# muzishen/IMAGHarmony

Hardware: AMD Instinct MI355X
Metric: 1024^2 SDXL images/sec (30 DDIM steps, PNS N seeds) (higher is better)
Workload: dtype bf16

## Files before the change

### imagharmony_amd/csrc/attention.hip

```cpp
#include "imh_attn_core.h"

namespace imh {

int g_attn_force_nw = 0;
int g_attn_mode = 0;
constexpr float ATT_DEFER_LOG2 = 8.0f;

template <typename T, int NW, int NPASS>
__global__ __launch_bounds__(64 * NW, (NPASS == 1 && NW == 4) ? 3 : 2) void attn_kernel(const AttnParams p) {
    constexpr int RND = 8 / NW;
    typedef typename Vec<T>::v8 v8;
    typedef typename Vec<T>::v4 v4;
    static_assert(32 * NW * 128 <= ATT_STAGES * 2 * ATT_TILE_BYTES, "Q/O staging must fit inside the ring");
    __shared__ __attribute__((aligned(16))) unsigned char smem[ATT_STAGES * 2 * ATT_TILE_BYTES];
    unsigned char* qs = smem;

    const int tid = threadIdx.x;
    const int lane = tid & 63;
    const int wave = __builtin_amdgcn_readfirstlane(tid >> 6);
    const int l32 = lane & 31;
    const int hi = lane >> 5;
    const int gx = (p.Lq + 32 * NW - 1) / (32 * NW);
    const int items = gx * p.H * p.B;
    const int per = (items + 7) >> 3;
    const int item = (blockIdx.x & 7) * per + (blockIdx.x >> 3);
    if ((int)(blockIdx.x >> 3) >= per || item >= items) return;
    const int hb = item / gx, qblk = item - hb * gx;
    const int b = hb / p.H, h = hb - b * p.H;
    const int q0 = qblk * (32 * NW);
    const int q = q0 + wave * 32 + l32;

    v8 qf[4];
    {
#pragma unroll
        for (int i = 0; i < 4; ++i) {
            const int row = wave * 32 + i * 8 + (lane >> 3);
            const int ch = stage_chunk_x(row, lane);
            const T* src = (const T*)p.Q + ((size_t)b * p.Lq + min(q0 + row, p.Lq - 1)) * p.ldq + h * 64 + ch * 8;
            glds16(src, qs + (wave * 32 + i * 8) * 128);
        }
        asm volatile("s_waitcnt vmcnt(0)" ::: "memory");
        const int row = wave * 32 + l32;
#pragma unroll
        for (int sd = 0; sd < 4; ++sd) qf[sd] = *(const v8*)(qs + tile_off(row, sd * 2 + hi, swz_x(row)));
        asm volatile("s_waitcnt lgkmcnt(0)" ::: "memory");
        __builtin_amdgcn_s_barrier();
    }

    f32x16 fin[2];
    attn_core<T, NW, NPASS>(p, smem, qf, b, h, wave, lane, item, fin);
    attn_store<T, NW>(p, qs, fin, b, h, q0, wave, lane);
    if (!ATT_TIMING) tail_prefetch(p.pf_ptr, p.pf_bytes, item, items, tid, 64 * NW);
}


template <typename T>
__global__ __launch_bounds__(256, 2) void attn_pipe_kernel(const AttnParams p) {
    constexpr int NW = 4;
    typedef typename Vec<T>::v8 v8;
    extern __shared__ __attribute__((aligned(16))) unsigned char smem[];
    unsigned char* qs = smem;
    const int tid = threadIdx.x;
    const int lane = tid & 63;
    const int wave = __builtin_amdgcn_readfirstlane(tid >> 6);
    const int l32 = lane & 31;
    const int hi = lane >> 5;
    const int gx = (p.Lq + 32 * NW - 1) / (32 * NW);
    const int items = gx * p.H * p.B;
    const int per = (items + 7) >> 3;
    const int split = p.split;
    const int jx = blockIdx.x >> 3;
    int item, qg = -1;
    if (jx < per - split) item = (blockIdx.x & 7) * per + jx;
    else {
        const int k = jx - (per - split);
        if (k >= 4 * split) return;
        item = (blockIdx.x & 7) * per + (per - split) + (k >> 2);
        qg = k & 3;
    }
    if (item >= items) return;
    const int hb = item / gx, qblk = item - hb * gx;
    const int b = hb / p.H, h = hb - b * p.H;
    const int q0 = qblk * (32 * NW);
#if ATT_TIMING == 2
    const unsigned long long ts_entry_ = __builtin_amdgcn_s_memrealtime();
#endif
    if (qg >= 0) {
        const float c = p.scale * LOG2E;
        unsigned char* my = smem + wave * (2 * ATT_TILE_BYTES);
        v8 qf[4];
        {
            const T* qrow = (const T*)p.Q + ((size_t)b * p.Lq + q0 + qg * 32 + l32) * p.ldq + h * 64 + hi * 8;
#pragma unroll
            for (int sd = 0; sd < 4; ++sd) qf[sd] = *(const v8*)(qrow + sd * 16);
        }
        f32x16 o[2];
#pragma unroll
        for (int dt = 0; dt < 2; ++dt)
#pragma unroll
            for (int r = 0; r < 16; ++r) o[dt][r] = 0.f;
        float m_run = NEG_BIG, l_run = 0.f;
        const int ntq = (p.Lk / ATT_KV) >> 2;
        const unsigned char* kq[2];
        const unsigned char* vq[2];
#pragma unroll
        for (int par = 0; par < 2; ++par) {
            const int row = par * 8 + (lane >> 3);
            const int ch = stage_chunk_x(row, lane);
            kq[par] = (const unsigned char*)((const T*)p.K + ((size_t)b * p.Lk_pad + row) * p.ldk + h * 64 + ch * 8);
            vq[par] = (const unsigned char*)((const T*)p.Vt + ((size_t)h * 64 + row) * p.ldvt + (size_t)b * p.Lk_pad + ch * 8);
        }
        const size_t kstep = (size_t)ATT_KV * p.ldk * sizeof(T), vstep = (size_t)ATT_KV * sizeof(T);
        const size_t krow16 = (size_t)16 * p.ldk * sizeof(T), vrow16 = (size_t)16 * p.ldvt * sizeof(T);
        for (int t = 0; t < ntq; ++t) {
            const int tile = wave * ntq + t;
#pragma unroll
            for (int i = 0; i < 2; ++i)
#pragma unroll
                for (int w = 0; w < 4; ++w) {
                    const int g16 = i * 2 + (w >> 1);
                    glds16(kq[w & 1] + tile * kstep + g16 * krow16, my + (i * 32 + w * 8) * 128);
                    glds16(vq[w & 1] + tile * vstep + g16 * vrow16, my + ATT_TILE_BYTES + (i * 32 + w * 8) * 128);
                }
            asm volatile("s_waitcnt vmcnt(0)" ::: "memory");
            attn_tile<T, false>(my, my + ATT_TILE_BYTES, qf, lane, tile * ATT_KV, p.Lk, c, o, m_run, l_run);
            asm volatile("s_waitcnt lgkmcnt(0)" ::: "memory");
        }
        const float l_tot = l_run + __shfl_xor(l_run, 32, 64);
        if (wave > 0) {
            float* w = (float*)my;
#pragma unroll
            for (int dt = 0; dt < 2; ++dt)
#pragma unroll
                for (int r = 0; r < 16; ++r) w[(dt * 16 + r) * 64 + lane] = o[dt][r];
            w[32 * 64 + lane] = m_run;
            w[33 * 64 + lane] = l_tot;
        }
        asm volatile("s_waitcnt lgkmcnt(0)" ::: "memory");
        __builtin_amdgcn_s_barrier();
        asm volatile("" ::: "memory");
        if (wave == 0) {
            float mi[4], li[4];
            mi[0] = m_run; li[0] = l_tot;
#pragma unroll
            for (int g = 1; g < 4; ++g) {
                const float* w = (const float*)(smem + g * (2 * ATT_TILE_BYTES));
                mi[g] = w[32 * 64 + lane]; li[g] = w[33 * 64 + lane];
            }
            const float m = fmaxf(fmaxf(mi[0], mi[1]), fmaxf(mi[2], mi[3]));
            float ai[4], den = 0.f;
#pragma unroll
            for (int g = 0; g < 4; ++g) { ai[g] = __builtin_amdgcn_exp2f((mi[g] - m) * c); den += li[g] * ai[g]; }
            const float inv = 1.0f / den;
            f32x16 fin[2];
#pragma unroll
            for (int dt = 0; dt < 2; ++dt)
#pragma unroll
                for (int r = 0; r < 16; ++r) {
                    float v = o[dt][r] * ai[0];
#pragma unroll
                    for (int g = 1; g < 4; ++g) v += ((const float*)(smem + g * (2 * ATT_TILE_BYTES)))[(dt * 16 + r) * 64 + lane] * ai[g];
                    fin[dt][r] = v * inv;
                }
            attn_store<T, 1>(p, smem, fin, b, h, q0 + qg * 32, 0, lane);
        }
#if ATT_TIMING == 2
        if (tid == 0 && p.pf_ptr) {
            asm volatile("s_waitcnt vmcnt(0)" ::: "memory");
            unsigned hwid;
            asm volatile("s_getreg_b32 %0, hwreg(HW_REG_HW_ID)" : "=s"(hwid));
            unsigned long long* dbg = (unsigned long long*)p.pf_ptr + (size_t)blockIdx.x * 4;
            dbg[0] = ts_entry_; dbg[1] = __builtin_amdgcn_s_memrealtime(); dbg[2] = hwid; dbg[3] = (blockIdx.x & 7) | 0x100;
        }
#else
        if (qg == 0) tail_prefetch(p.pf_ptr, p.pf_bytes, item, items, tid, 64 * NW);
#endif
        return;
    }
    v8 qf[4];
    {
#pragma unroll
        for (int i = 0; i < 4; ++i) {
            const int row = wave * 32 + i * 8 + (lane >> 3);
            const int ch = stage_chunk_x(row, lane);
            const T* src = (const T*)p.Q + ((size_t)b * p.Lq + min(q0 + row, p.Lq - 1)) * p.ldq + h * 64 + ch * 8;
            glds16(src, qs + (wave * 32 + i * 8) * 128);
        }
        asm volatile("s_waitcnt vmcnt(0)" ::: "memory");
        const int row = wave * 32 + l32;
#pragma unroll
        for (int sd = 0; sd < 4; ++sd) qf[sd] = *(const v8*)(qs + tile_off(row, sd * 2 + hi, swz_x(row)));
        asm volatile("s_waitcnt lgkmcnt(0)" ::: "memory");
        __builtin_amdgcn_s_barrier();
    }
    f32x16 fin[2];
    attn_core_pipe<T>(p, smem, qf, b, h, wave, lane, fin);
    attn_store<T, NW>(p, qs, fin, b, h, q0, wave, lane);
#if ATT_TIMING == 2
    if (tid == 0 && p.pf_ptr) {
        asm volatile("s_waitcnt vmcnt(0)" ::: "memory");
        unsigned hwid;
        asm volatile("s_getreg_b32 %0, hwreg(HW_REG_HW_ID)" : "=s"(hwid));
        unsigned long long* dbg = (unsigned long long*)p.pf_ptr + (size_t)blockIdx.x * 4;
        dbg[0] = ts_entry_; dbg[1] = __builtin_amdgcn_s_memrealtime(); dbg[2] = hwid; dbg[3] = blockIdx.x & 7;
    }
#else
    tail_prefetch(p.pf_ptr, p.pf_bytes, item, items, tid, 64 * NW);
#endif
}

#ifdef IMH_EXPERIMENTAL
template <typename T>
__global__ __launch_bounds__(512, 4) void attn_ks_kernel(const AttnParams p) {
    typedef typename Vec<T>::v8 v8;
    extern __shared__ __attribute__((aligned(16))) unsigned char smem[];
    const int tid = threadIdx.x;
    const int lane = tid & 63;
    const int wave = __builtin_amdgcn_readfirstlane(tid >> 6);
    const int g = wave >> 2, qg = wave & 3;
    const int hi = lane >> 5;
    const int gx = (p.Lq + 127) / 128;
    const int items = gx * p.H * p.B;
    const int per = (items + 7) >> 3;
    const int item = (blockIdx.x & 7) * per + (blockIdx.x >> 3);
    if ((int)(blockIdx.x >> 3) >= per || item >= items) return;
    const int hb = item / gx, qblk = item - hb * gx;
    const int b = hb / p.H, h = hb - b * p.H;
    const int q0 = qblk * 128;
    v8 qf[4];
    {
        const T* qrow = (const T*)p.Q + ((size_t)b * p.Lq + min(q0 + qg * 32 + (lane & 31), p.Lq - 1)) * p.ldq + h * 64 + hi * 8;
#pragma unroll
        for (int sd = 0; sd < 4; ++sd) qf[sd] = *(const v8*)(qrow + sd * 16);
    }
    f32x16 o[2], fin[2];
    float m_run, l_run;
    attn_core_ks<T>(p, smem + g * (2 * 2 * ATT_TILE_BYTES), qf, b, h, g, qg, lane, o, m_run, l_run);
    asm volatile("s_waitcnt lgkmcnt(0)" ::: "memory");
    __builtin_amdgcn_s_barrier();
    attn_ks_merge((float*)smem, p.scale * LOG2E, g, qg, lane, o, m_run, l_run, fin);
    if (g == 0) attn_store<T, 4>(p, smem + 4 * 34 * 64 * 4, fin, b, h, q0, qg, lane);
    else tail_prefetch(p.pf_ptr, p.pf_bytes, item, items, tid - 256, 256);
}
#endif

template <typename T>
__global__ __launch_bounds__(256) void attn_small_kernel(const SmallAttnParams p) {
    extern __shared__ float sm[];
    float* sc = sm;
    float* qrow = sm + p.Lk;
    float* red = qrow + p.dq;
    const int b = blockIdx.x / p.H, h = blockIdx.x % p.H;
    const int tid = threadIdx.x;
    const T* Q = (const T*)p.Q + (size_t)b * p.Lq * p.ldq + h * p.dq;
    const T* K = (const T*)p.K + (size_t)b * p.Lk * p.ldk + h * p.dq;
    const T* V = (const T*)p.V + (size_t)b * p.Lk * p.ldv + h * p.dv;
    T* O = (T*)p.O + (size_t)b * p.Lq * p.ldo + h * p.dv;
    for (int i = 0; i < p.Lq; ++i) {
        for (int d = tid; d < p.dq; d += 256) qrow[d] = to_f32(Q[(size_t)i * p.ldq + d]);
        __syncthreads();
        float mx = -1e30f;
        for (int k = tid; k < p.Lk; k += 256) {
            const T* kr = K + (size_t)k * p.ldk;
            float s = 0.f;
            for (int d = 0; d < p.dq; ++d) s += qrow[d] * to_f32(kr[d]);
            s *= p.scale;
            sc[k] = s;
            mx = fmaxf(mx, s);
        }
        mx = wave_max(mx);
        if ((tid & 63) == 0) red[tid >> 6] = mx;
        __syncthreads();
        mx = fmaxf(fmaxf(red[0], red[1]), fmaxf(red[2], red[3]));
        float sum = 0.f;
        for (int k = tid; k < p.Lk; k += 256) { const float e = __expf(sc[k] - mx); sc[k] = e; sum += e; }
        sum = wave_sum(sum);
        if ((tid & 63) == 0) red[4 + (tid >> 6)] = sum;
        __syncthreads();
        sum = red[4] + red[5] + red[6] + red[7];
// ... 55 lines not shown
        for (int k0 = 0; k0 < LkP; k0 += 64) {
            const int k = k0 + lane;
            const float e = k < p.Lk ? __expf(mypr[k] - mx) : 0.f;
            mypr[k] = e;
            sum += e;
        }
        sum = wave_sum(sum);
        __builtin_amdgcn_wave_barrier();
        const float inv = 1.0f / sum;
        for (int d = lane; d < p.dv; d += 64) {
            float o = 0.f;
            for (int k = 0; k < p.Lk; ++k) o += mypr[k] * to_f32(vs[(size_t)k * p.dv + d]);
            O[(size_t)q * p.ldo + d] = from_f32<T>(o * inv);
        }
        __builtin_amdgcn_wave_barrier();
    }
}

int attention_small_launch(const SmallAttnParams& p, int dtype, hipStream_t stream) {
    if (p.B <= 0 || p.H <= 0 || p.Lq <= 0 || p.Lk <= 0 || p.dq <= 0 || p.dv <= 0 || p.Lk > 8192 || p.dq > 1024) {
        set_error("attention_small: unsupported shape"); return IMH_ERR_SHAPE;
    }
    if (dtype != IMH_DT_BF16 && dtype != IMH_DT_F16) { set_error("attention_small: unknown dtype %d", dtype); return IMH_ERR_DTYPE; }
    {
        const int LkP = (p.Lk + 63) & ~63;
        const size_t need = ((size_t)p.dq * LkP + (size_t)p.Lk * p.dv) * 2 + (size_t)(4 * LkP + 4 * p.dq) * sizeof(float);
        const bool aligned = !(p.dq & 7) && !(p.dv & 7) && !(p.ldk & 7) && !(p.ldv & 7) && !(((size_t)p.Lk * p.dv * 2 + (size_t)p.dq * LkP * 2) & 15);
        if (aligned && need <= 150 * 1024) {
            dim3 grid(p.B * p.H);
            if (dtype == IMH_DT_BF16) {
                static DynLdsOnce a0;
                a0.ensure((const void*)attn_small_lds_kernel<bf16_t>, 150 * 1024);
                hipLaunchKernelGGL((attn_small_lds_kernel<bf16_t>), grid, dim3(256), need, stream, p, LkP);
            } else {
                static DynLdsOnce a1;
                a1.ensure((const void*)attn_small_lds_kernel<f16_t>, 150 * 1024);
                hipLaunchKernelGGL((attn_small_lds_kernel<f16_t>), grid, dim3(256), need, stream, p, LkP);
            }
            return check_launch("attn_small_lds_kernel");
        }
    }
    const size_t lds = (size_t)(p.Lk + p.dq + 8) * sizeof(float);
    dim3 grid(p.B * p.H);
    if (dtype == IMH_DT_BF16) hipLaunchKernelGGL((attn_small_kernel<bf16_t>), grid, dim3(256), lds, stream, p);
    else if (dtype == IMH_DT_F16) hipLaunchKernelGGL((attn_small_kernel<f16_t>), grid, dim3(256), lds, stream, p);
    else { set_error("attention_small: unknown dtype %d", dtype); return IMH_ERR_DTYPE; }
    return check_launch("attn_small_kernel");
}

int attention_launch(const AttnParams& p, int dtype, hipStream_t stream) {
    if (p.Lk <= 0 || p.Lk_pad % ATT_KV != 0 || p.Lk_pad < p.Lk) {
        set_error("attention: Lk=%d Lk_pad=%d (pad must be a multiple of 64 and >= Lk)", p.Lk, p.Lk_pad);
        return IMH_ERR_SHAPE;
    }
    if (p.K2 && (p.Lk2 <= 0 || p.Lk2_pad % ATT_KV != 0 || p.Lk2_pad < p.Lk2)) {
        set_error("attention: Lk2=%d Lk2_pad=%d invalid", p.Lk2, p.Lk2_pad);
        return IMH_ERR_SHAPE;
    }
    if ((p.ldq & 7) || (p.ldk & 7) || (p.ldvt & 7) || (p.ldo & 7) || (p.K2 && ((p.ldk2 & 7) || (p.ldvt2 & 7)))) {
        set_error("attention: leading dimensions must be multiples of 8 elements");
        return IMH_ERR_SHAPE;
    }
    if (p.B <= 0 || p.H <= 0 || p.Lq <= 0) { set_error("attention: empty problem"); return IMH_ERR_SHAPE; }
    if (dtype != IMH_DT_BF16 && dtype != IMH_DT_F16) { set_error("attention: unknown dtype %d", dtype); return IMH_ERR_DTYPE; }
    constexpr int nw = 4;
    const int items = ((p.Lq + 32 * nw - 1) / (32 * nw)) * p.H * p.B;
    dim3 grid(8 * ((items + 7) / 8));
    if (!p.K2 && p.Lk % (2 * ATT_KV) == 0 && p.Lk >= 4 * ATT_KV && (g_attn_mode == 5 || g_attn_mode == 6)) {
#ifndef IMH_EXPERIMENTAL
        return experimental_refused("the key-split attention kernel (imh_debug_set(4, 5 | 6))");
#else
        const int lds = 2 * 2 * 2 * ATT_TILE_BYTES;
        const int items128 = ((p.Lq + 127) / 128) * p.H * p.B;
        dim3 grid2(8 * ((items128 + 7) / 8));
        AttnParams q = p;
        q.defer_log2 = g_attn_mode == 6 ? 0.0f : ATT_DEFER_LOG2;
        if (dtype == IMH_DT_BF16) { static DynLdsOnce once; once.ensure((const void*)attn_ks_kernel<bf16_t>, lds);
                                    hipLaunchKernelGGL((attn_ks_kernel<bf16_t>), grid2, dim3(512), lds, stream, q); }
        else { static DynLdsOnce once; once.ensure((const void*)attn_ks_kernel<f16_t>, lds);
               hipLaunchKernelGGL((attn_ks_kernel<f16_t>), grid2, dim3(512), lds, stream, q); }
        return check_launch("attn_ks_kernel");
#endif
    }
    if (!p.K2 && p.Lk % ATT_KV == 0 && (g_attn_mode == 2 || g_attn_mode == 3 || g_attn_mode == 7 || (g_attn_mode == 0 && p.Lk >= 4 * ATT_KV))) {
        const int lds = ATT_PIPE_STAGES * 2 * ATT_TILE_BYTES;
        AttnParams q = p;
        q.defer_log2 = g_attn_mode == 2 ? 0.0f : ATT_DEFER_LOG2;
        const int per = (items + 7) / 8;
        q.split = (g_attn_mode != 7 && per > 32 && per % 32 != 0 && per % 32 <= 16 && p.Lq % 128 == 0 && p.Lk % (4 * ATT_KV) == 0) ? per % 32 : 0;
        dim3 gridp(8 * (per + 3 * q.split));
        if (dtype == IMH_DT_BF16) { static DynLdsOnce once; once.ensure((const void*)attn_pipe_kernel<bf16_t>, lds);
                                    hipLaunchKernelGGL((attn_pipe_kernel<bf16_t>), gridp, dim3(256), lds, stream, q); }
        else { static DynLdsOnce once; once.ensure((const void*)attn_pipe_kernel<f16_t>, lds);
               hipLaunchKernelGGL((attn_pipe_kernel<f16_t>), gridp, dim3(256), lds, stream, q); }
        return check_launch("attn_pipe_kernel");
    }
#define IMH_ATT_LAUNCH(TT, NWV) do { if (p.K2) hipLaunchKernelGGL((attn_kernel<TT, NWV, 2>), grid, dim3(64 * NWV), 0, stream, p); \
        else hipLaunchKernelGGL((attn_kernel<TT, NWV, 1>), grid, dim3(64 * NWV), 0, stream, p); } while (0)
    if (dtype == IMH_DT_BF16) IMH_ATT_LAUNCH(bf16_t, 4);
    else IMH_ATT_LAUNCH(f16_t, 4);
#undef IMH_ATT_LAUNCH
    return check_launch("attn_kernel");
}

}
```

### imagharmony_amd/csrc/imh_attn_core.h

```cpp
#pragma once
#include "imh_common.h"
#include "imh_kernels.h"
#include <type_traits>

namespace imh {

constexpr int ATT_KV = 64;
constexpr int ATT_TILE_BYTES = 64 * 128;
constexpr int ATT_STAGES = 3;
constexpr float LOG2E = 1.4426950408889634f;
constexpr float NEG_BIG = -1.0e30f;

typedef __attribute__((ext_vector_type(2))) float f32x2;
__device__ __forceinline__ float max3f(float a, float b, float c) {
    float r;
    asm("v_max3_f32 %0, %1, %2, %3" : "=v"(r) : "v"(a), "v"(b), "v"(c));
    return r;
}
__device__ __forceinline__ float mfma_first_max(float a, float b) { return __builtin_fmaxf(a, b); }
__device__ __forceinline__ float xhalf_max(float x) {
    const unsigned u = __builtin_bit_cast(unsigned, x);
    auto r = __builtin_amdgcn_permlane32_swap(u, u, false, false);
    return fmaxf(__builtin_bit_cast(float, (unsigned)r[0]), __builtin_bit_cast(float, (unsigned)r[1]));
}
#ifndef ATT_ABL
#define ATT_ABL 0
#endif
#define ATT_EXP2(x) ((ATT_ABL & 9) ? (x) : __builtin_amdgcn_exp2f(x))
#ifndef ATT_TIMING
#define ATT_TIMING 0
#endif
#if ATT_TIMING
#define ATT_TICK(i) do { asm volatile("s_nop 0" ::: "memory"); const unsigned long long tn_ = __builtin_readcyclecounter(); tacc[i] += tn_ - tm0; tm0 = tn_; } while (0)
#else
#define ATT_TICK(i) do {} while (0)
#endif


template <typename T, bool MASK, int NKT>
__device__ __forceinline__ void attn_tile_n(const unsigned char* ks, const unsigned char* vs, const typename Vec<T>::v8 (&qf)[4],
                                            const int lane, const int kbase, const int Lk, const float c, f32x16 (&o)[2],
                                            float& m_run, float& l_run);

template <typename T, int NW, int NPASS>
__device__ __forceinline__ void attn_core(const AttnParams& p, unsigned char* smem, const typename Vec<T>::v8 (&qf)[4],
                                          const int b, const int h, const int wave, const int lane, const int item,
                                          f32x16 (&fin)[2]) {
    constexpr int RND = 8 / NW;
    typedef typename Vec<T>::v8 v8;
    const int tid = threadIdx.x;
    const int hi = lane >> 5;
    (void)tid; (void)item;
    const float c = p.scale * LOG2E;

#pragma unroll
    for (int dt = 0; dt < 2; ++dt)
#pragma unroll
        for (int r = 0; r < 16; ++r) fin[dt][r] = 0.f;

#pragma unroll
    for (int pass = 0; pass < NPASS; ++pass) {
        const T* Kp = (const T*)(pass == 0 ? p.K : p.K2);
        const T* Vp = (const T*)(pass == 0 ? p.Vt : p.Vt2);
        const int Lk = pass == 0 ? p.Lk : p.Lk2;
        const int Lkp = pass == 0 ? p.Lk_pad : p.Lk2_pad;
        const int ldk = pass == 0 ? p.ldk : p.ldk2;
        const int ldvt = pass == 0 ? p.ldvt : p.ldvt2;
        const float wgt = pass == 0 ? 1.0f : (p.scale2_tab ? p.scale2_tab[*p.step] : p.scale2);
        const int ntiles = (Lk + ATT_KV - 1) / ATT_KV;

        auto stage = [&](int buf, int tile) {
            unsigned char* ks = smem + buf * 2 * ATT_TILE_BYTES;
            unsigned char* vs = ks + ATT_TILE_BYTES;
            const int kbase = tile * ATT_KV;
#pragma unroll
            for (int i = 0; i < RND; ++i) {
                const int row = i * (NW * 8) + wave * 8 + (lane >> 3);
                const int ch = stage_chunk_x(row, lane);
                const T* ksrc = Kp + ((size_t)b * Lkp + kbase + row) * ldk + h * 64 + ch * 8;
                glds16(ksrc, ks + (i * (NW * 8) + wave * 8) * 128);
                const T* vsrc = Vp + ((size_t)h * 64 + row) * ldvt + (size_t)b * Lkp + kbase + ch * 8;
                glds16(vsrc, vs + (i * (NW * 8) + wave * 8) * 128);
            }
        };

        f32x16 o[2];
#pragma unroll
        for (int dt = 0; dt < 2; ++dt)
#pragma unroll
            for (int r = 0; r < 16; ++r) o[dt][r] = 0.f;
        float m_run = NEG_BIG, l_run = 0.f;

        constexpr int LPT = 2 * RND;
#pragma unroll
        for (int s = 0; s < ATT_STAGES - 1; ++s)
            if (s < ntiles) stage(s, s);
        int cur = 0;
#if ATT_TIMING
        unsigned long long tacc[5] = {0, 0, 0, 0, 0}, tm0 = __builtin_readcyclecounter();
#endif
        for (int t = 0; t < ntiles; ++t) {
            if (ATT_ABL & 16) {
            } else if (t + ATT_STAGES - 2 < ntiles) asm volatile("s_waitcnt vmcnt(%0)" ::"n"((ATT_STAGES - 2) * LPT) : "memory");
            else asm volatile("s_waitcnt vmcnt(0)" ::: "memory");
            if (!(ATT_ABL & 4)) __builtin_amdgcn_s_barrier();
            asm volatile("" ::: "memory");
// ... 145 lines not shown
        for (int s = 0; s < 2; ++s)
#pragma unroll
            for (int dt = 0; dt < 2; ++dt) vf[kt][s][dt] = *(const v8*)(vs + att_v_off(lane, dt, kt, s));
    __builtin_amdgcn_sched_barrier(0);
    if (ragged) {
#pragma unroll
        for (int kt = 0; kt < NKT; ++kt)
#pragma unroll
            for (int r = 0; r < 16; ++r)
                if (kbase + kt * 32 + st_key(r, hi) >= Lk) st[kt][r] = NEG_BIG;
    }
    float mx;
    if constexpr (NKT == 2) {
        mx = max3f(mfma_first_max(st[0][0], st[1][0]), st[0][1], st[1][1]);
        mx = fmaxf(mx, st[0][2]);
#pragma unroll
        for (int r = 2; r < 15; ++r) mx = max3f(mx, st[1][r], st[0][r + 1]);
        mx = fmaxf(mx, st[1][15]);
    } else {
        mx = max3f(mfma_first_max(st[0][0], st[0][1]), st[0][2], st[0][3]);
#pragma unroll
        for (int r = 4; r < 16; r += 2) mx = max3f(mx, st[0][r], st[0][r + 1]);
    }
    mx = xhalf_max(mx);
    const float m_new = fmaxf(m_run, mx);
    const f32x2 c2 = {c, c};
    const f32x2 nmc2 = {-m_new * c, -m_new * c};
    f32x2 ps2 = {0.f, 0.f};
    v8 pf[NKT][2];
#pragma unroll
    for (int kt = 0; kt < NKT; ++kt)
#pragma unroll
        for (int r = 0; r < 16; r += 2) {
            const f32x2 s2 = {st[kt][r], st[kt][r + 1]};
            const f32x2 e2 = __builtin_elementwise_fma(s2, c2, nmc2);
            const f32x2 p2 = {__builtin_amdgcn_exp2f(e2[0]), __builtin_amdgcn_exp2f(e2[1])};
            ps2 += p2;
            pf[kt][r >> 3][r & 7] = from_f32<T>(p2[0]);
            pf[kt][r >> 3][(r & 7) + 1] = from_f32<T>(p2[1]);
        }
    if (__any(m_new != m_run)) {
        const float alpha = __builtin_amdgcn_exp2f((m_run - m_new) * c);
        l_run *= alpha;
#pragma unroll
        for (int dt = 0; dt < 2; ++dt)
#pragma unroll
            for (int r = 0; r < 16; ++r) o[dt][r] *= alpha;
        m_run = m_new;
    }
    l_run += ps2[0] + ps2[1];
    __builtin_amdgcn_sched_barrier(0);
#pragma unroll
    for (int kt = 0; kt < NKT; ++kt)
#pragma unroll
        for (int s = 0; s < 2; ++s)
#pragma unroll
            for (int dt = 0; dt < 2; ++dt) o[dt] = mfma32(vf[kt][s][dt], pf[kt][s], o[dt]);
}

template <typename T, bool MASK = true>
__device__ __forceinline__ void attn_tile(const unsigned char* ks, const unsigned char* vs, const typename Vec<T>::v8 (&qf)[4],
                                          const int lane, const int kbase, const int Lk, const float c, f32x16 (&o)[2],
                                          float& m_run, float& l_run) {
    if (MASK && kbase + 32 >= Lk) attn_tile_n<T, MASK, 1>(ks, vs, qf, lane, kbase, Lk, c, o, m_run, l_run);
    else attn_tile_n<T, MASK, 2>(ks, vs, qf, lane, kbase, Lk, c, o, m_run, l_run);
}

template <typename T>
__device__ __forceinline__ void attn_stage_tile(const T* Kp, const T* Vp, const int Lkp, const int ldk, const int ldvt, const int b,
                                                const int h, const int tile, unsigned char* ks, unsigned char* vs, const int wave,
                                                const int lane) {
    const int kbase = tile * ATT_KV;
#pragma unroll
    for (int i = 0; i < 2; ++i) {
        const int row = i * 32 + wave * 8 + (lane >> 3);
        const int ch = stage_chunk_x(row, lane);
        glds16(Kp + ((size_t)b * Lkp + kbase + row) * ldk + h * 64 + ch * 8, ks + (i * 32 + wave * 8) * 128);
        glds16(Vp + ((size_t)h * 64 + row) * ldvt + (size_t)b * Lkp + kbase + ch * 8, vs + (i * 32 + wave * 8) * 128);
    }
}

constexpr int ATT_PIPE_STAGES = 4;

template <typename T>
__device__ __forceinline__ void attn_core_pipe(const AttnParams& p, unsigned char* smem, const typename Vec<T>::v8 (&qf)[4],
                                               const int b, const int h, const int wave, const int lane, f32x16 (&fin)[2]) {
    typedef typename Vec<T>::v8 v8;
    constexpr int S = ATT_PIPE_STAGES, LPT = 4;
    const int hi = lane >> 5;
    const float c = p.scale * LOG2E;
    const T* Kp = (const T*)p.K;
    const T* Vp = (const T*)p.Vt;
    const int Lk = p.Lk;
    const int ntiles = (Lk + ATT_KV - 1) / ATT_KV;
    auto stage = [&](int tile) {
        unsigned char* ks = smem + (tile & (S - 1)) * 2 * ATT_TILE_BYTES;
        attn_stage_tile<T>(Kp, Vp, p.Lk_pad, p.ldk, p.ldvt, b, h, tile, ks, ks + ATT_TILE_BYTES, wave, lane);
    };
    const int srow = wave * 8 + (lane >> 3);
    const unsigned char* ksrc[2];
    const unsigned char* vsrc[2];
#pragma unroll
    for (int i = 0; i < 2; ++i) {
        const int row = i * 32 + srow;
        const int ch = stage_chunk_x(row, lane);
        ksrc[i] = (const unsigned char*)(Kp + ((size_t)b * p.Lk_pad + row) * p.ldk + h * 64 + ch * 8);
        vsrc[i] = (const unsigned char*)(Vp + ((size_t)h * 64 + row) * p.ldvt + (size_t)b * p.Lk_pad + ch * 8);
    }
    const size_t kstep = (size_t)ATT_KV * p.ldk * sizeof(T), vstep = (size_t)ATT_KV * sizeof(T);
    auto stage_piece = [&](int tile, int q) {
        unsigned char* ks = smem + (tile & (S - 1)) * 2 * ATT_TILE_BYTES;
        const int i = q >> 1;
        if (q & 1) glds16(vsrc[i] + (size_t)tile * vstep, ks + ATT_TILE_BYTES + (i * 32 + wave * 8) * 128);
        else glds16(ksrc[i] + (size_t)tile * kstep, ks + (i * 32 + wave * 8) * 128);
    };
    f32x16 o[2];
#pragma unroll
    for (int dt = 0; dt < 2; ++dt)
#pragma unroll
        for (int r = 0; r < 16; ++r) o[dt][r] = 0.f;
    float m_run = NEG_BIG, l_run = 0.f;

    auto qk = [&](f32x16 (&st)[2], const unsigned char* ks) {
        v8 kf[2][4];
#pragma unroll
        for (int kt = 0; kt < 2; ++kt)
#pragma unroll
            for (int sd = 0; sd < 4; ++sd) kf[kt][sd] = *(const v8*)(ks + att_k_off(lane, kt, sd));
#pragma unroll
        for (int kt = 0; kt < 2; ++kt) {
#pragma unroll
            for (int r = 0; r < 16; ++r) st[kt][r] = 0.f;
#pragma unroll
            for (int sd = 0; sd < 4; ++sd) st[kt] = mfma32(kf[kt][sd], qf[sd], st[kt]);
        }
    };
    auto rowmax = [&](f32x16 (&st)[2], const int tile) -> float {
        (void)tile; (void)hi;
        float mx = max3f(mfma_first_max(st[0][0], st[1][0]), st[0][1], st[1][1]);
        mx = fmaxf(mx, st[0][2]);
#pragma unroll
        for (int r = 2; r < 15; ++r) mx = max3f(mx, st[1][r], st[0][r + 1]);
        mx = fmaxf(mx, st[1][15]);
        return xhalf_max(mx);
    };
    const float defer = p.defer_log2;
    auto rescale = [&](const float m_new) {
        if (__any((m_new - m_run) * c > defer)) {
            const float alpha = __builtin_amdgcn_exp2f((m_run - m_new) * c);
            l_run *= alpha;
#pragma unroll
            for (int dt = 0; dt < 2; ++dt)
#pragma unroll
                for (int r = 0; r < 16; ++r) o[dt][r] *= alpha;
            m_run = m_new;
        }
    };

#pragma unroll
    for (int s = 0; s < S - 1; ++s)
        if (s < ntiles) stage(s);
    if (ntiles >= 3) asm volatile("s_waitcnt vmcnt(%0)" ::"n"(2 * LPT) : "memory");
    else if (ntiles == 2) asm volatile("s_waitcnt vmcnt(%0)" ::"n"(LPT) : "memory");
    else asm volatile("s_waitcnt vmcnt(0)" ::: "memory");
    __builtin_amdgcn_s_barrier();
    asm volatile("" ::: "memory");
    f32x16 stA[2], stB[2];
    qk(stA, smem);
    rescale(fmaxf(m_run, rowmax(stA, 0)));

    auto iter = [&](auto HN, auto STG, f32x16 (&cur)[2], f32x16 (&nxt)[2], const int t) {
        constexpr bool has_next = decltype(HN)::value;
        constexpr int stg = decltype(STG)::value;
        const bool stage_more = stg == 1 || (stg == 2 && has_next && t + 3 < ntiles);
        if (has_next) {
            if (t + 2 < ntiles) asm volatile("s_waitcnt vmcnt(%0)" ::"n"(LPT) : "memory");
            else asm volatile("s_waitcnt vmcnt(0)" ::: "memory");
            __builtin_amdgcn_s_barrier();
            asm volatile("" ::: "memory");
        }
        const unsigned char* vs = smem + (t & (S - 1)) * 2 * ATT_TILE_BYTES + ATT_TILE_BYTES;
        const unsigned char* ksn = smem + ((t + 1) & (S - 1)) * 2 * ATT_TILE_BYTES;
        v8 kf[2][4], vf[2][2][2];
        if (has_next) {
#pragma unroll
            for (int sd = 0; sd < 4; ++sd)
#pragma unroll
                for (int kt = 0; kt < 2; ++kt) kf[kt][sd] = *(const v8*)(ksn + att_k_off(lane, kt, sd));
        }
        auto v_reads = [&]() {
#pragma unroll
            for (int kt = 0; kt < 2; ++kt)
#pragma unroll
                for (int s2 = 0; s2 < 2; ++s2)
#pragma unroll
                    for (int dt = 0; dt < 2; ++dt) vf[kt][s2][dt] = *(const v8*)(vs + att_v_off(lane, dt, kt, s2));
        };
        if (!has_next) v_reads();
        __builtin_amdgcn_sched_barrier(0);
        const f32x2 c2 = {c, c};
        const f32x2 nmc2 = {-m_run * c, -m_run * c};
        f32x2 ps2 = {0.f, 0.f};
        v8 pf[2][2];
        auto p_chunk = [&](auto J) {
            constexpr int j = decltype(J)::value;
            constexpr int kt = j >> 2, r0 = (j & 3) * 4;
#pragma unroll
            for (int r = r0; r < r0 + 4; r += 2) {
                const f32x2 s2 = {cur[kt][r], cur[kt][r + 1]};
                const f32x2 e2 = __builtin_elementwise_fma(s2, c2, nmc2);
                const f32x2 p2 = {__builtin_amdgcn_exp2f(e2[0]), __builtin_amdgcn_exp2f(e2[1])};
                ps2 += p2;
                pf[kt][r >> 3][r & 7] = from_f32<T>(p2[0]);
                pf[kt][r >> 3][(r & 7) + 1] = from_f32<T>(p2[1]);
            }
        };
        auto b_step = [&](auto J) {
            constexpr int j = decltype(J)::value;
            constexpr int sd = j >> 1, kt = j & 1;
            p_chunk(J);
            if constexpr (j == 3) { if (has_next) v_reads(); }
            __builtin_amdgcn_sched_barrier(0);
            if (has_next) {
                if constexpr (sd == 0) {
#pragma unroll
                    for (int r = 0; r < 16; ++r) nxt[kt][r] = 0.f;
                }
                nxt[kt] = mfma32(kf[kt][sd], qf[sd], nxt[kt]);
                __builtin_amdgcn_sched_barrier(0);
            }
        };
        b_step(std::integral_constant<int, 0>{}); b_step(std::integral_constant<int, 1>{});
        b_step(std::integral_constant<int, 2>{}); b_step(std::integral_constant<int, 3>{});
        b_step(std::integral_constant<int, 4>{}); b_step(std::integral_constant<int, 5>{});
        b_step(std::integral_constant<int, 6>{}); b_step(std::integral_constant<int, 7>{});
        l_run += ps2[0] + ps2[1];
        float mx = NEG_BIG;
        __builtin_amdgcn_sched_barrier(0);
        auto a_step = [&](auto J) {
            constexpr int j = decltype(J)::value;
            constexpr int kt = j >> 2, s2 = (j >> 1) & 1, dt = j & 1;
            o[dt] = mfma32(vf[kt][s2][dt], pf[kt][s2], o[dt]);
            __builtin_amdgcn_sched_barrier(0);
            if (has_next) {
                constexpr int k2 = j >> 2, r0 = (j & 3) * 4;
                if constexpr ((j & 3) == 0) mx = max3f(mfma_first_max(mx, nxt[k2][r0]), nxt[k2][r0 + 1], nxt[k2][r0 + 2]);
                else mx = max3f(mx, nxt[k2][r0], nxt[k2][r0 + 1]);
                if constexpr ((j & 3) == 0) mx = fmaxf(mx, nxt[k2][r0 + 3]);
                else mx = max3f(mx, nxt[k2][r0 + 2], nxt[k2][r0 + 3]);
                if constexpr (j >= 2 && j < 6 && stg != 0) {
                    if (stage_more) stage_piece(t + 3, j - 2);
                }
            }
            __builtin_amdgcn_sched_barrier(0);
        };
        a_step(std::integral_constant<int, 0>{}); a_step(std::integral_constant<int, 1>{});
        a_step(std::integral_constant<int, 2>{}); a_step(std::integral_constant<int, 3>{});
        a_step(std::integral_constant<int, 4>{}); a_step(std::integral_constant<int, 5>{});
        a_step(std::integral_constant<int, 6>{}); a_step(std::integral_constant<int, 7>{});
        if (has_next) rescale(fmaxf(m_run, xhalf_max(mx)));
        asm volatile("" ::: "memory");
    };
    const std::integral_constant<bool, true> YES{};
    const std::integral_constant<bool, false> NO{};
    const std::integral_constant<int, 0> STG_NONE{};
    const std::integral_constant<int, 1> STG_ALWAYS{};
    const std::integral_constant<int, 2> STG_CHECK{};
    int t = 0;
    for (; t + 4 < ntiles; t += 2) {
        iter(YES, STG_ALWAYS, stA, stB, t);
        iter(YES, STG_ALWAYS, stB, stA, t + 1);
    }
    for (; t + 2 < ntiles; t += 2) {
        iter(YES, STG_CHECK, stA, stB, t);
        iter(YES, STG_CHECK, stB, stA, t + 1);
    }
    if (t + 1 < ntiles) {
        iter(YES, STG_NONE, stA, stB, t);
        iter(NO, STG_NONE, stB, stA, t + 1);
    } else {
        iter(NO, STG_NONE, stA, stB, t);
    }

    __builtin_amdgcn_s_barrier();
    const float inv = 1.0f / (l_run + __shfl_xor(l_run, 32, 64));
#pragma unroll
    for (int dt = 0; dt < 2; ++dt)
#pragma unroll
        for (int r = 0; r < 16; ++r) fin[dt][r] = o[dt][r] * inv;
}

template <typename T>
__device__ __forceinline__ void attn_core_ks(const AttnParams& p, unsigned char* gs, const typename Vec<T>::v8 (&qf)[4],
                                             const int b, const int h, const int g, const int qg, const int lane,
                                             f32x16 (&o)[2], float& m_run, float& l_run) {
    typedef typename Vec<T>::v8 v8;
    const int hi = lane >> 5;
    (void)hi;
    const float c = p.scale * LOG2E;
    const float defer = p.defer_log2;
    const T* Kp = (const T*)p.K;
    const T* Vp = (const T*)p.Vt;
    const int tg = (p.Lk / ATT_KV) >> 1;
    const int t0 = g * tg;
#pragma unroll
    for (int dt = 0; dt < 2; ++dt)
#pragma unroll
        for (int r = 0; r < 16; ++r) o[dt][r] = 0.f;
    m_run = NEG_BIG; l_run = 0.f;
    const unsigned char* ksrc[2];
    const unsigned char* vsrc[2];
#pragma unroll
    for (int i = 0; i < 2; ++i) {
        const int row = i * 32 + qg * 8 + (lane >> 3);
        const int ch = stage_chunk_x(row, lane);
        ksrc[i] = (const unsigned char*)(Kp + ((size_t)b * p.Lk_pad + row) * p.ldk + h * 64 + ch * 8);
        vsrc[i] = (const unsigned char*)(Vp + ((size_t)h * 64 + row) * p.ldvt + (size_t)b * p.Lk_pad + ch * 8);
    }
    const size_t kstep = (size_t)ATT_KV * p.ldk * sizeof(T), vstep = (size_t)ATT_KV * sizeof(T);
    auto stage = [&](int slot, int tile) {
        unsigned char* ks = gs + slot * 2 * ATT_TILE_BYTES;
#pragma unroll
        for (int i = 0; i < 2; ++i) {
            glds16(ksrc[i] + tile * kstep, ks + (i * 32 + qg * 8) * 128);
            glds16(vsrc[i] + tile * vstep, ks + ATT_TILE_BYTES + (i * 32 + qg * 8) * 128);
        }
    };
    stage(0, t0);
    for (int t = 0; t < tg; ++t) {
        asm volatile("s_waitcnt vmcnt(0)" ::: "memory");
        __builtin_amdgcn_s_barrier();
        asm volatile("" ::: "memory");
        if (t + 1 < tg) stage((t + 1) & 1, t0 + t + 1);
        const unsigned char* ks = gs + (t & 1) * 2 * ATT_TILE_BYTES;
        const unsigned char* vs = ks + ATT_TILE_BYTES;
        f32x16 st[2];
#pragma unroll
        for (int kt = 0; kt < 2; ++kt) {
            v8 kf[4];
#pragma unroll
            for (int sd = 0; sd < 4; ++sd) kf[sd] = *(const v8*)(ks + att_k_off(lane, kt, sd));
#pragma unroll
            for (int r = 0; r < 16; ++r) st[kt][r] = 0.f;
#pragma unroll
            for (int sd = 0; sd < 4; ++sd) st[kt] = mfma32(kf[sd], qf[sd], st[kt]);
        }
        float mx = max3f(mfma_first_max(st[0][0], st[1][0]), st[0][1], st[1][1]);
        mx = fmaxf(mx, st[0][2]);
#pragma unroll
        for (int r = 2; r < 15; ++r) mx = max3f(mx, st[1][r], st[0][r + 1]);
        mx = fmaxf(mx, st[1][15]);
        mx = xhalf_max(mx);
        const float m_new = fmaxf(m_run, mx);
        if (__any((m_new - m_run) * c > defer)) {
            const float alpha = __builtin_amdgcn_exp2f((m_run - m_new) * c);
            l_run *= alpha;
#pragma unroll
            for (int dt = 0; dt < 2; ++dt)
#pragma unroll
                for (int r = 0; r < 16; ++r) o[dt][r] *= alpha;
            m_run = m_new;
        }
        const f32x2 c2 = {c, c};
        const f32x2 nmc2 = {-m_run * c, -m_run * c};
// ... 90 lines not shown
```

Measured before the change: 1.726.

## Add lean attention pipe path with buffer loads, static ring slots, cheaper max

Adds a LEAN variant of the pipelined attention kernel that stages K/V tiles into LDS through buffer-resource loads with 32-bit offsets instead of 64-bit pointer arithmetic. The main loop is unrolled by four so ring-slot indices become compile-time constants, and the running row max uses fmed3-based max that skips NaN canonicalisation. The aim is fewer scalar and vector address instructions and fewer ALU ops per tile. It is gated on tensor sizes fitting in 31-bit offsets and can be disabled via mode 8. It adds more template instantiations and code size.

```diff
diff --git a/imagharmony_amd/csrc/attention.hip b/imagharmony_amd/csrc/attention.hip
--- a/imagharmony_amd/csrc/attention.hip
+++ b/imagharmony_amd/csrc/attention.hip
@@ -54,7 +54,7 @@
 }
 
 
-template <typename T>
+template <typename T, bool LEAN>
 __global__ __launch_bounds__(256, 2) void attn_pipe_kernel(const AttnParams p) {
     constexpr int NW = 4;
     typedef typename Vec<T>::v8 v8;
@@ -194,7 +194,7 @@
         __builtin_amdgcn_s_barrier();
     }
     f32x16 fin[2];
-    attn_core_pipe<T>(p, smem, qf, b, h, wave, lane, fin);
+    attn_core_pipe<T, LEAN>(p, smem, qf, b, h, wave, lane, fin);
     attn_store<T, NW>(p, qs, fin, b, h, q0, wave, lane);
 #if ATT_TIMING == 2
     if (tid == 0 && p.pf_ptr) {
@@ -416,17 +416,19 @@
         return check_launch("attn_ks_kernel");
 #endif
     }
-    if (!p.K2 && p.Lk % ATT_KV == 0 && (g_attn_mode == 2 || g_attn_mode == 3 || g_attn_mode == 7 || (g_attn_mode == 0 && p.Lk >= 4 * ATT_KV))) {
+    if (!p.K2 && p.Lk % ATT_KV == 0 && (g_attn_mode == 2 || g_attn_mode == 3 || g_attn_mode == 7 || ((g_attn_mode == 0 || g_attn_mode == 8) && p.Lk >= 4 * ATT_KV))) {
         const int lds = ATT_PIPE_STAGES * 2 * ATT_TILE_BYTES;
+        const bool lean = g_attn_mode != 8 && (size_t)p.Lk_pad * p.ldk * 2 < (1u << 31) && (size_t)64 * p.ldvt * 2 < (1u << 31);
         AttnParams q = p;
         q.defer_log2 = g_attn_mode == 2 ? 0.0f : ATT_DEFER_LOG2;
         const int per = (items + 7) / 8;
         q.split = (g_attn_mode != 7 && per > 32 && per % 32 != 0 && per % 32 <= 16 && p.Lq % 128 == 0 && p.Lk % (4 * ATT_KV) == 0) ? per % 32 : 0;
         dim3 gridp(8 * (per + 3 * q.split));
-        if (dtype == IMH_DT_BF16) { static DynLdsOnce once; once.ensure((const void*)attn_pipe_kernel<bf16_t>, lds);
-                                    hipLaunchKernelGGL((attn_pipe_kernel<bf16_t>), gridp, dim3(256), lds, stream, q); }
-        else { static DynLdsOnce once; once.ensure((const void*)attn_pipe_kernel<f16_t>, lds);
-               hipLaunchKernelGGL((attn_pipe_kernel<f16_t>), gridp, dim3(256), lds, stream, q); }
+#define IMH_ATT_PIPE(TT, LN) do { static DynLdsOnce once; once.ensure((const void*)attn_pipe_kernel<TT, LN>, lds); \
+        hipLaunchKernelGGL((attn_pipe_kernel<TT, LN>), gridp, dim3(256), lds, stream, q); } while (0)
+        if (dtype == IMH_DT_BF16) { if (lean) IMH_ATT_PIPE(bf16_t, true); else IMH_ATT_PIPE(bf16_t, false); }
+        else { if (lean) IMH_ATT_PIPE(f16_t, true); else IMH_ATT_PIPE(f16_t, false); }
+#undef IMH_ATT_PIPE
         return check_launch("attn_pipe_kernel");
     }
 #define IMH_ATT_LAUNCH(TT, NWV) do { if (p.K2) hipLaunchKernelGGL((attn_kernel<TT, NWV, 2>), grid, dim3(64 * NWV), 0, stream, p); \
diff --git a/imagharmony_amd/csrc/imh_attn_core.h b/imagharmony_amd/csrc/imh_attn_core.h
--- a/imagharmony_amd/csrc/imh_attn_core.h
+++ b/imagharmony_amd/csrc/imh_attn_core.h
@@ -18,10 +18,17 @@
     return r;
 }
 __device__ __forceinline__ float mfma_first_max(float a, float b) { return __builtin_fmaxf(a, b); }
+__device__ __forceinline__ float max_nc(float a, float b) { return __builtin_amdgcn_fmed3f(a, b, 3.40282347e38f); }
+__device__ __forceinline__ float mfma_first_max_nc(float a, float b) { return max_nc(a, b); }
 __device__ __forceinline__ float xhalf_max(float x) {
     const unsigned u = __builtin_bit_cast(unsigned, x);
     auto r = __builtin_amdgcn_permlane32_swap(u, u, false, false);
     return fmaxf(__builtin_bit_cast(float, (unsigned)r[0]), __builtin_bit_cast(float, (unsigned)r[1]));
+}
+__device__ __forceinline__ float xhalf_max_nc(float x) {
+    const unsigned u = __builtin_bit_cast(unsigned, x);
+    auto r = __builtin_amdgcn_permlane32_swap(u, u, false, false);
+    return max_nc(__builtin_bit_cast(float, (unsigned)r[0]), __builtin_bit_cast(float, (unsigned)r[1]));
 }
 #ifndef ATT_ABL
 #define ATT_ABL 0
@@ -333,7 +340,7 @@
 
 constexpr int ATT_PIPE_STAGES = 4;
 
-template <typename T>
+template <typename T, bool LEAN>
 __device__ __forceinline__ void attn_core_pipe(const AttnParams& p, unsigned char* smem, const typename Vec<T>::v8 (&qf)[4],
                                                const int b, const int h, const int wave, const int lane, f32x16 (&fin)[2]) {
     typedef typename Vec<T>::v8 v8;
@@ -359,12 +366,37 @@
         vsrc[i] = (const unsigned char*)(Vp + ((size_t)h * 64 + row) * p.ldvt + (size_t)b * p.Lk_pad + ch * 8);
     }
     const size_t kstep = (size_t)ATT_KV * p.ldk * sizeof(T), vstep = (size_t)ATT_KV * sizeof(T);
-    auto stage_piece = [&](int tile, int q) {
-        unsigned char* ks = smem + (tile & (S - 1)) * 2 * ATT_TILE_BYTES;
+    __amdgpu_buffer_rsrc_t krs, vrs;
+    int kvo[2], vvo[2];
+    if constexpr (LEAN) {
+        const int bu = __builtin_amdgcn_readfirstlane(b), hu = __builtin_amdgcn_readfirstlane(h);
+        const T* kb = Kp + (size_t)bu * p.Lk_pad * p.ldk + hu * 64;
+        const T* vb = Vp + (size_t)hu * 64 * p.ldvt + (size_t)bu * p.Lk_pad;
+        krs = __builtin_amdgcn_make_buffer_rsrc((void*)kb, (short)0, (int)(((p.Lk_pad - 1) * p.ldk + 64) * (int)sizeof(T)), 0x00020000);
+        vrs = __builtin_amdgcn_make_buffer_rsrc((void*)vb, (short)0, (int)((63 * p.ldvt + p.Lk_pad) * (int)sizeof(T)), 0x00020000);
+#pragma unroll
+        for (int i = 0; i < 2; ++i) {
+            const int row = i * 32 + srow;
+            const int ch = stage_chunk_x(row, lane);
+            kvo[i] = (row * p.ldk + ch * 8) * (int)sizeof(T);
+            vvo[i] = (row * p.ldvt + ch * 8) * (int)sizeof(T);
+        }
+    }
+    const int kstep32 = ATT_KV * p.ldk * (int)sizeof(T);
+    auto stage_piece_at = [&](int slot, int tile, int q) {
+        unsigned char* ks = smem + slot * 2 * ATT_TILE_BYTES;
         const int i = q >> 1;
-        if (q & 1) glds16(vsrc[i] + (size_t)tile * vstep, ks + ATT_TILE_BYTES + (i * 32 + wave * 8) * 128);
-        else glds16(ksrc[i] + (size_t)tile * kstep, ks + (i * 32 + wave * 8) * 128);
+        if constexpr (LEAN) {
+            typedef __attribute__((address_space(3))) void* lds_ptr;
+            if (q & 1) __builtin_amdgcn_raw_ptr_buffer_load_lds(vrs, (lds_ptr)(ks + ATT_TILE_BYTES + (i * 32 + wave * 8) * 128), 16, vvo[i],
+                                                                tile * (ATT_KV * (int)sizeof(T)), 0, 0);
+            else __builtin_amdgcn_raw_ptr_buffer_load_lds(krs, (lds_ptr)(ks + (i * 32 + wave * 8) * 128), 16, kvo[i], tile * kstep32, 0, 0);
+        } else {
+            if (q & 1) glds16(vsrc[i] + (size_t)tile * vstep, ks + ATT_TILE_BYTES + (i * 32 + wave * 8) * 128);
+            else glds16(ksrc[i] + (size_t)tile * kstep, ks + (i * 32 + wave * 8) * 128);
+        }
     };
+    auto stage_piece = [&](int tile, int q) { stage_piece_at(tile & (S - 1), tile, q); };
     f32x16 o[2];
 #pragma unroll
     for (int dt = 0; dt < 2; ++dt)
@@ -410,7 +442,12 @@
 
 #pragma unroll
     for (int s = 0; s < S - 1; ++s)
-        if (s < ntiles) stage(s);
+        if (s < ntiles) {
+            if constexpr (LEAN) {
+#pragma unroll
+                for (int q = 0; q < 4; ++q) stage_piece(s, q);
+            } else stage(s);
+        }
     if (ntiles >= 3) asm volatile("s_waitcnt vmcnt(%0)" ::"n"(2 * LPT) : "memory");
     else if (ntiles == 2) asm volatile("s_waitcnt vmcnt(%0)" ::"n"(LPT) : "memory");
     else asm volatile("s_waitcnt vmcnt(0)" ::: "memory");
@@ -420,9 +457,10 @@
     qk(stA, smem);
     rescale(fmaxf(m_run, rowmax(stA, 0)));
 
-    auto iter = [&](auto HN, auto STG, f32x16 (&cur)[2], f32x16 (&nxt)[2], const int t) {
+    auto iter = [&](auto HN, auto STG, f32x16 (&cur)[2], f32x16 (&nxt)[2], const int t, auto SL) {
         constexpr bool has_next = decltype(HN)::value;
         constexpr int stg = decltype(STG)::value;
+        constexpr int sl = decltype(SL)::value;
         const bool stage_more = stg == 1 || (stg == 2 && has_next && t + 3 < ntiles);
         if (has_next) {
             if (t + 2 < ntiles) asm volatile("s_waitcnt vmcnt(%0)" ::"n"(LPT) : "memory");
@@ -430,8 +468,9 @@
             __builtin_amdgcn_s_barrier();
             asm volatile("" ::: "memory");
         }
-        const unsigned char* vs = smem + (t & (S - 1)) * 2 * ATT_TILE_BYTES + ATT_TILE_BYTES;
-        const unsigned char* ksn = smem + ((t + 1) & (S - 1)) * 2 * ATT_TILE_BYTES;
+        const int slot = sl >= 0 ? sl : (t & (S - 1));
+        const unsigned char* vs = smem + slot * 2 * ATT_TILE_BYTES + ATT_TILE_BYTES;
+        const unsigned char* ksn = smem + ((slot + 1) & (S - 1)) * 2 * ATT_TILE_BYTES;
         v8 kf[2][4], vf[2][2][2];
         if (has_next) {
 #pragma unroll
@@ -495,12 +534,22 @@
             __builtin_amdgcn_sched_barrier(0);
             if (has_next) {
                 constexpr int k2 = j >> 2, r0 = (j & 3) * 4;
-                if constexpr ((j & 3) == 0) mx = max3f(mfma_first_max(mx, nxt[k2][r0]), nxt[k2][r0 + 1], nxt[k2][r0 + 2]);
-                else mx = max3f(mx, nxt[k2][r0], nxt[k2][r0 + 1]);
-                if constexpr ((j & 3) == 0) mx = fmaxf(mx, nxt[k2][r0 + 3]);
-                else mx = max3f(mx, nxt[k2][r0 + 2], nxt[k2][r0 + 3]);
+                if constexpr (LEAN && j == 0) {
+                    mx = max3f(mfma_first_max_nc(nxt[k2][r0], nxt[k2][r0 + 1]), nxt[k2][r0 + 2], nxt[k2][r0 + 3]);
+                } else if constexpr (LEAN && j == 4) {
+                    mx = max3f(mx, mfma_first_max_nc(nxt[k2][r0], nxt[k2][r0 + 1]), nxt[k2][r0 + 2]);
+                    mx = max3f(mx, nxt[k2][r0 + 3], nxt[k2][r0 + 3]);
+                } else {
+                    if constexpr ((j & 3) == 0) mx = max3f(mfma_first_max(mx, nxt[k2][r0]), nxt[k2][r0 + 1], nxt[k2][r0 + 2]);
+                    else mx = max3f(mx, nxt[k2][r0], nxt[k2][r0 + 1]);
+                    if constexpr ((j & 3) == 0) mx = fmaxf(mx, nxt[k2][r0 + 3]);
+                    else mx = max3f(mx, nxt[k2][r0 + 2], nxt[k2][r0 + 3]);
+                }
                 if constexpr (j >= 2 && j < 6 && stg != 0) {
-                    if (stage_more) stage_piece(t + 3, j - 2);
+                    if (stage_more) {
+                        if constexpr (sl >= 0) stage_piece_at((sl + 3) & (S - 1), t + 3, j - 2);
+                        else stage_piece(t + 3, j - 2);
+                    }
                 }
             }
             __builtin_amdgcn_sched_barrier(0);
@@ -509,7 +558,10 @@
         a_step(std::integral_constant<int, 2>{}); a_step(std::integral_constant<int, 3>{});
         a_step(std::integral_constant<int, 4>{}); a_step(std::integral_constant<int, 5>{});
         a_step(std::integral_constant<int, 6>{}); a_step(std::integral_constant<int, 7>{});
-        if (has_next) rescale(fmaxf(m_run, xhalf_max(mx)));
+        if (has_next) {
+            if constexpr (LEAN) rescale(max_nc(m_run, xhalf_max_nc(mx)));
+            else rescale(fmaxf(m_run, xhalf_max(mx)));
+        }
         asm volatile("" ::: "memory");
     };
     const std::integral_constant<bool, true> YES{};
@@ -517,20 +569,30 @@
     const std::integral_constant<int, 0> STG_NONE{};
     const std::integral_constant<int, 1> STG_ALWAYS{};
     const std::integral_constant<int, 2> STG_CHECK{};
+    const std::integral_constant<int, -1> SLX{};
     int t = 0;
-    for (; t + 4 < ntiles; t += 2) {
-        iter(YES, STG_ALWAYS, stA, stB, t);
-        iter(YES, STG_ALWAYS, stB, stA, t + 1);
+    if constexpr (LEAN) {
+        for (; t + 6 < ntiles; t += 4) {
+            iter(YES, STG_ALWAYS, stA, stB, t, std::integral_constant<int, 0>{});
+            iter(YES, STG_ALWAYS, stB, stA, t + 1, std::integral_constant<int, 1>{});
+            iter(YES, STG_ALWAYS, stA, stB, t + 2, std::integral_constant<int, 2>{});
+            iter(YES, STG_ALWAYS, stB, stA, t + 3, std::integral_constant<int, 3>{});
+        }
+    } else {
+        for (; t + 4 < ntiles; t += 2) {
+            iter(YES, STG_ALWAYS, stA, stB, t, SLX);
+            iter(YES, STG_ALWAYS, stB, stA, t + 1, SLX);
+        }
     }
     for (; t + 2 < ntiles; t += 2) {
-        iter(YES, STG_CHECK, stA, stB, t);
-        iter(YES, STG_CHECK, stB, stA, t + 1);
+        iter(YES, STG_CHECK, stA, stB, t, SLX);
+        iter(YES, STG_CHECK, stB, stA, t + 1, SLX);
     }
     if (t + 1 < ntiles) {
-        iter(YES, STG_NONE, stA, stB, t);
-        iter(NO, STG_NONE, stB, stA, t + 1);
+        iter(YES, STG_NONE, stA, stB, t, SLX);
+        iter(NO, STG_NONE, stB, stA, t + 1, SLX);
     } else {
-        iter(NO, STG_NONE, stA, stB, t);
+        iter(NO, STG_NONE, stA, stB, t, SLX);
     }
 
     __builtin_amdgcn_s_barrier();
```

Measured after the change: 1.736 (median of 6 runs). About the same (+0.6%).
